# CompVis/stable-diffusion

Measured on AMD Instinct MI355X. Metric: 512x512 images/sec, SD-v1-4 50-step PLMS CFG=7.5, higher is better.
Workload: dtype f16

## Files before the change

### include/sdmi.h

```cpp
#ifndef SDMI_H_
#define SDMI_H_

#include <stdint.h>

#ifdef __cplusplus
extern "C" {
#endif

#define SDMI_ABI_VERSION 17

typedef struct sdmi_unet sdmi_unet;

typedef struct sdmi_unet_cfg {
  int32_t in_channels;
  int32_t out_channels;
  int32_t model_channels;
  int32_t num_res_blocks;
  int32_t n_levels;
  int32_t channel_mult[8];
  int32_t n_attention_resolutions;
  int32_t attention_resolutions[8];
  int32_t num_heads;
  int32_t transformer_depth;
  int32_t context_dim;
// ... 111 lines not shown
  void* pgn_out; int32_t pgn_keep_f32; int32_t* pgn_applied;
  void* out_lo;
} sdmi_igemm_desc;
int sdmi_k_igemm(const sdmi_igemm_desc* d, void* stream);
int sdmi_k_ff_tail(const sdmi_igemm_desc* proj_out, const void* ln_f16, const float* lnp, float ln_eps, const float* csd,
                   const void* wgg_f16, const void* wff2_f16, const float* bff2, const float* t, void* stream);
int sdmi_k_st_tail(const sdmi_igemm_desc* proj_out, const void* a_f16, const void* wo_f16, const float* bo, float* t, const float* ln_gamma,
                   float ln_eps, const float* csd, const void* wgg_f16, const void* wff2_f16, const float* bff2, void* stream);
int sdmi_k_gn_conv3(const sdmi_igemm_desc* conv, const float* x0, const float* x1, int c0, int c1, float* gn_ws, int64_t gn_ws_floats,
                    const float* gn_gamma, const float* gn_beta, float gn_eps, void* stream);
int sdmi_k_st_head(const float* x, float* gn_ws, int64_t gn_ws_floats, const float* gn_gamma, const float* gn_beta, float gn_eps,
                   const void* w_in3, const float* b_in, float* t, const float* ln_gamma, float ln_eps, const void* wqkv_f16,
                   const float* lnf_cs, const float* lnf_d, void* q, void* k, void* vt, int B, int ntok, int ntok_pad, int heads, int dh,
                   int C, void* stream);
int sdmi_k_st_mid(const void* a_f16, const void* wo_f16, const float* bo, float* t, const float* ln_gamma, float ln_eps, const void* wq_f16,
                  const float* lnf_cs, const float* lnf_d, void* q, int B, int ntok, int heads, int dh, int C, void* stream);
int sdmi_k_st_mid_ctx(const void* a_f16, const void* wo_f16, const float* bo, float* t, const float* ln_gamma, float ln_eps, const void* wq_f16,
                      const float* lnf_cs, const float* lnf_d, const void* ctx_k, const void* ctx_vt, int nkv, int nkv_pad, float scale, void* ao_out,
                      int B, int ntok, int heads, int dh, int C, void* stream);
int sdmi_k_ln_fold_prep(const void* w_f16, int N, int K, int ldw, const float* gamma, const float* beta, const float* bias,
                        float* cs, float* d, void* stream);
int sdmi_k_attention(const void* q, const void* k, const void* vt, void* out, int BH, int heads, int nq, int nkv,
                     int nkv_pad, int d, float scale, void* stream);
int sdmi_k_attention_ctx(const void* x, const void* wq, const void* k, const void* vt, void* out, int BH, int heads, int nq,
                         int nkv, int nkv_pad, int d, float scale, const float* lnf_part, float lnf_eps, const float* lnf_cs,
                         const float* lnf_d, void* stream);
int sdmi_k_attention_split16(const void* q, const void* q_lo, const void* k, const void* k_lo, const void* vt, const void* vt_lo, void* out,
                             void* out_lo, int BH, int heads, int nq, int nkv, int nkv_pad, int d, float scale, void* stream);
int sdmi_k_attention_causal(const void* q, const void* k, const void* vt, void* out, int BH, int heads, int n, int n_pad,
                            int d, float scale, void* stream);
int sdmi_k_groupnorm(const float* x0, const float* x1, int c0, int c1, int B, int HW, const float* gamma,
                     const float* beta, float eps, int silu, void* out_f16, float* out_f32, void* raw_f16, void* out_lo,
                     void* raw_lo, float* partial_ws, int64_t partial_floats, void* stream);
int64_t sdmi_k_groupnorm_ws_floats(int B, int HW);
int sdmi_k_conv3gn(const float* x0, const float* x1, int c0, int c1, int B, int H, int W, const float* gamma,
                   const float* beta, float eps, const void* w_packed, int N, const float* bias, const float* rowvec,
                   int ld_rowvec, const float* residual, int ldr, float* out, int ldo, int splitk, float* splitk_ws,
                   int64_t splitk_ws_floats, float* gn_ws, int64_t gn_ws_floats, int tile, void* raw_hi, void* raw_lo,
                   void* stream);
int sdmi_k_layernorm(const float* x, const float* gamma, const float* beta, void* out_f16, int M, int C, float eps,
                     void* stream);
int sdmi_k_cast_f16(const float* x, void* out_f16, void* out_lo, int64_t n, void* stream);
int sdmi_k_split_heads(const float* src, int ld, int col0, void* dst, void* dst_lo, int kind, int B, int ntok, int ntok_pad, int heads, int dh,
                       void* stream);
int sdmi_k_geglu_split(const float* src, int M, int F, void* out, void* out_lo, void* stream);
int sdmi_k_layernorm_split(const float* x, const float* gamma, const float* beta, void* out, void* out_lo, int M, int C, float eps, void* stream);
// ... 31 lines not shown
```

### stable-diffusion_amd/_lib.py

```python
import ctypes as C
import os

_HERE = os.path.dirname(os.path.abspath(__file__))
LIB_PATH = os.environ.get('SDMI_LIB_PATH') or os.path.join(_HERE, 'libsdmi.so')

c_f32p = C.c_void_p
c_ptr = C.c_void_p


class UNetCfg(C.Structure):
    _fields_ = [('in_channels', C.c_int32), ('out_channels', C.c_int32), ('model_channels', C.c_int32),
                ('num_res_blocks', C.c_int32), ('n_levels', C.c_int32), ('channel_mult', C.c_int32 * 8),
                ('n_attention_resolutions', C.c_int32), ('attention_resolutions', C.c_int32 * 8),
                ('num_heads', C.c_int32), ('transformer_depth', C.c_int32), ('context_dim', C.c_int32)]


class VaeCfg(C.Structure):
    _fields_ = [('ch', C.c_int32), ('out_ch', C.c_int32), ('n_levels', C.c_int32), ('ch_mult', C.c_int32 * 8),
                ('num_res_blocks', C.c_int32), ('in_channels', C.c_int32), ('z_channels', C.c_int32),
                ('embed_dim', C.c_int32)]


class ClipCfg(C.Structure):
    _fields_ = [('vocab_size', C.c_int32), ('hidden_size', C.c_int32), ('intermediate_size', C.c_int32),
# ... 66 lines not shown
    'sdmi_clip_set_weight': (C.c_int, [c_ptr, C.c_char_p, c_ptr, C.POINTER(C.c_int64), C.c_int, c_ptr]),
    'sdmi_clip_finalize': (C.c_int, [c_ptr]),
    'sdmi_clip_workspace_bytes': (C.c_int64, [c_ptr, C.c_int, C.c_int]),
    'sdmi_clip_forward': (C.c_int, [c_ptr, c_ptr, c_ptr, C.c_int, C.c_int, c_ptr, C.c_int64, c_ptr]),
    'sdmi_has_experiments': (C.c_int, []),
    'sdmi_k_igemm': (C.c_int, [C.POINTER(IGemmDesc), c_ptr]),
    'sdmi_k_ff_tail': (C.c_int, [C.POINTER(IGemmDesc), c_ptr, c_ptr, C.c_float, c_ptr, c_ptr, c_ptr, c_ptr, c_ptr, c_ptr]),
    'sdmi_k_gn_conv3': (C.c_int, [C.POINTER(IGemmDesc), c_ptr, c_ptr, C.c_int, C.c_int, c_ptr, C.c_int64, c_ptr, c_ptr, C.c_float, c_ptr]),
    'sdmi_k_st_mid_ctx': (C.c_int, [c_ptr, c_ptr, c_ptr, c_ptr, c_ptr, C.c_float, c_ptr, c_ptr, c_ptr, c_ptr, c_ptr, C.c_int, C.c_int, C.c_float, c_ptr,
                                    C.c_int, C.c_int, C.c_int, C.c_int, C.c_int, c_ptr]),
    'sdmi_k_st_tail': (C.c_int, [C.POINTER(IGemmDesc), c_ptr, c_ptr, c_ptr, c_ptr, c_ptr, C.c_float, c_ptr, c_ptr, c_ptr, c_ptr, c_ptr]),
    'sdmi_k_st_mid': (C.c_int, [c_ptr, c_ptr, c_ptr, c_ptr, c_ptr, C.c_float, c_ptr, c_ptr, c_ptr, c_ptr, C.c_int, C.c_int, C.c_int, C.c_int,
                                C.c_int, c_ptr]),
    'sdmi_k_st_head': (C.c_int, [c_ptr, c_ptr, C.c_int64, c_ptr, c_ptr, C.c_float, c_ptr, c_ptr, c_ptr, c_ptr, C.c_float, c_ptr, c_ptr, c_ptr,
                                 c_ptr, c_ptr, c_ptr, C.c_int, C.c_int, C.c_int, C.c_int, C.c_int, C.c_int, c_ptr]),
    'sdmi_k_attention_split16': (C.c_int, [c_ptr, c_ptr, c_ptr, c_ptr, c_ptr, c_ptr, c_ptr, c_ptr, C.c_int, C.c_int, C.c_int, C.c_int,
                                           C.c_int, C.c_int, C.c_float, c_ptr]),
    'sdmi_k_attention_causal': (C.c_int, [c_ptr, c_ptr, c_ptr, c_ptr, C.c_int, C.c_int, C.c_int, C.c_int, C.c_int, C.c_float,
                                          c_ptr]),
    'sdmi_k_pointwise_nchw': (C.c_int, [c_ptr, c_ptr, c_ptr, c_ptr, C.c_int, C.c_int, C.c_int, C.c_int, C.c_float, c_ptr]),
    'sdmi_k_softmax_rows': (C.c_int, [c_ptr, c_ptr, C.c_int, C.c_int, C.c_float, c_ptr]),
    'sdmi_k_attention': (C.c_int, [c_ptr, c_ptr, c_ptr, c_ptr, C.c_int, C.c_int, C.c_int, C.c_int, C.c_int, C.c_int,
                                   C.c_float, c_ptr]),
    'sdmi_k_groupnorm': (C.c_int, [c_ptr, c_ptr, C.c_int, C.c_int, C.c_int, C.c_int, c_ptr, c_ptr, C.c_float, C.c_int,
                                   c_ptr, c_ptr, c_ptr, c_ptr, c_ptr, c_ptr, C.c_int64, c_ptr]),
    'sdmi_k_groupnorm_ws_floats': (C.c_int64, [C.c_int, C.c_int]),
    'sdmi_k_conv3gn': (C.c_int, [c_ptr, c_ptr, C.c_int, C.c_int, C.c_int, C.c_int, C.c_int, c_ptr, c_ptr, C.c_float, c_ptr,
                                 C.c_int, c_ptr, c_ptr, C.c_int, c_ptr, C.c_int, c_ptr, C.c_int, C.c_int, c_ptr, C.c_int64,
                                 c_ptr, C.c_int64, C.c_int, c_ptr, c_ptr, c_ptr]),
    'sdmi_k_layernorm': (C.c_int, [c_ptr, c_ptr, c_ptr, c_ptr, C.c_int, C.c_int, C.c_float, c_ptr]),
    'sdmi_k_cast_f16': (C.c_int, [c_ptr, c_ptr, c_ptr, C.c_int64, c_ptr]),
    'sdmi_k_split_heads': (C.c_int, [c_ptr, C.c_int, C.c_int, c_ptr, c_ptr, C.c_int, C.c_int, C.c_int, C.c_int, C.c_int, C.c_int,
                                     c_ptr]),
    'sdmi_k_geglu_split': (C.c_int, [c_ptr, C.c_int, C.c_int, c_ptr, c_ptr, c_ptr]),
    'sdmi_k_layernorm_split': (C.c_int, [c_ptr, c_ptr, c_ptr, c_ptr, c_ptr, C.c_int, C.c_int, C.c_float, c_ptr]),
    'sdmi_k_timestep_embedding': (C.c_int, [c_ptr, c_ptr, c_ptr, C.c_int, C.c_int, c_ptr]),
    'sdmi_k_small_linear': (C.c_int, [c_ptr, C.c_int, c_ptr, c_ptr, c_ptr, C.c_int, C.c_int, C.c_int, C.c_int,
                                      C.c_int, c_ptr]),
    'sdmi_k_conv_in': (C.c_int, [c_ptr, c_ptr, c_ptr, c_ptr, C.c_int, C.c_int, C.c_int, C.c_int, C.c_int, c_ptr]),
    'sdmi_k_conv_out': (C.c_int, [c_ptr, c_ptr, c_ptr, c_ptr, C.c_int, C.c_int, C.c_int, C.c_int, C.c_int, c_ptr]),
    'sdmi_k_pack_conv_weight': (C.c_int, [c_ptr, c_ptr, C.c_int, C.c_int, C.c_int, C.c_int, c_ptr]),
    'sdmi_k_pack_conv_out': (C.c_int, [c_ptr, c_ptr, C.c_int, C.c_int, c_ptr]),
    'sdmi_k_pack_split3': (C.c_int, [c_ptr, c_ptr, C.c_int, C.c_int, c_ptr]),
    'sdmi_k_pack_geglu': (C.c_int, [c_ptr, c_ptr, c_ptr, c_ptr, C.c_int, C.c_int, c_ptr]),
    'sdmi_k_attention_ctx': (C.c_int, [c_ptr, c_ptr, c_ptr, c_ptr, c_ptr, C.c_int, C.c_int, C.c_int, C.c_int, C.c_int, C.c_int, C.c_float,
                                       c_ptr, C.c_float, c_ptr, c_ptr, c_ptr]),
# ... 55 lines not shown
```

### stable-diffusion_amd/csrc/api.cpp

```cpp
#include <string.h>

#include <new>

#include "prof.h"
#include "split16.h"
#include "unet.h"
#include "vae.h"
#include "clip.h"

namespace sdmi {
static thread_local std::string g_err;
void set_error(const std::string& msg) { g_err = msg; }
int fail(const std::string& msg) { g_err = msg; return -1; }
}

struct sdmi_unet { sdmi::UNet impl; };
struct sdmi_vae { sdmi::Vae impl; };
struct sdmi_clip { sdmi::ClipText impl; };

using namespace sdmi;

static void* g_zero_page[16] = {nullptr};
static int zero_page(const f16** out) {
  int dev = 0;
// ... 323 lines not shown
int sdmi_k_st_mid_ctx(const void* a_f16, const void* wo_f16, const float* bo, float* t, const float* ln_gamma, float ln_eps, const void* wq_f16,
                      const float* lnf_cs, const float* lnf_d, const void* ctx_k, const void* ctx_vt, int nkv, int nkv_pad, float scale, void* ao_out,
                      int B, int ntok, int heads, int dh, int C, void* stream) {
  StHeadParams p = StHeadParams();
  p.a16 = (const f16*)a_f16; p.w_in = (const f16*)wo_f16; p.b_in = bo; p.t = t; p.ln_gamma = ln_gamma; p.ln_eps = ln_eps;
  p.wqkv = (const f16*)wq_f16; p.lnf_cs = lnf_cs; p.lnf_d = lnf_d;
  p.ctx_k = (const f16*)ctx_k; p.ctx_vt = (const f16*)ctx_vt; p.ctx_nkv = nkv; p.ctx_nkv_pad = nkv_pad; p.ctx_scale = scale; p.ao_out = (f16*)ao_out;
  SDMI_CHECK(ctx_k && ctx_vt && ao_out, "st_mid_ctx: null argument");
  p.M = B * ntok; p.B = B; p.ntok = ntok; p.ntok_pad = ntok; p.heads = heads; p.dh = dh; p.C = C;
  return launch_st_mid(p, (hipStream_t)stream);
}
int sdmi_k_ln_fold_prep(const void* w_f16, int N, int K, int ldw, const float* gamma, const float* beta, const float* bias,
                        float* cs, float* d, void* stream) {
  return launch_ln_fold_prep((const f16*)w_f16, N, K, ldw, gamma, beta, bias, cs, d, (hipStream_t)stream);
}
int sdmi_k_attention(const void* q, const void* k, const void* vt, void* out, int BH, int heads, int nq, int nkv,
                     int nkv_pad, int d, float scale, void* stream) {
  AttnParams a = AttnParams();
  a.q = (const f16*)q; a.k = (const f16*)k; a.vt = (const f16*)vt; a.out = (f16*)out;
  a.BH = BH; a.heads = heads; a.nq = nq; a.nkv = nkv; a.nkv_pad = nkv_pad; a.d = d; a.scale = scale;
  if (const char* e = getenv("SDMI_ATTN_NW")) a.nw = atoi(e);
  return launch_attention(a, (hipStream_t)stream);
}
int sdmi_k_attention_split16(const void* q, const void* q_lo, const void* k, const void* k_lo, const void* vt, const void* vt_lo, void* out,
                             void* out_lo, int BH, int heads, int nq, int nkv, int nkv_pad, int d, float scale, void* stream) {
  AttnSplitParams a = AttnSplitParams();
  a.q = (const f16*)q; a.q_lo = (const f16*)q_lo; a.k = (const f16*)k; a.k_lo = (const f16*)k_lo; a.vt = (const f16*)vt;
  a.vt_lo = (const f16*)vt_lo; a.out = (f16*)out; a.out_lo = (f16*)out_lo;
  a.BH = BH; a.heads = heads; a.nq = nq; a.nkv = nkv; a.nkv_pad = nkv_pad; a.d = d; a.scale = scale;
  return launch_attention_split16(a, (hipStream_t)stream);
}
int sdmi_k_attention_ctx(const void* x, const void* wq, const void* k, const void* vt, void* out, int BH, int heads, int nq,
                         int nkv, int nkv_pad, int d, float scale, const float* lnf_part, float lnf_eps, const float* lnf_cs,
                         const float* lnf_d, void* stream) {
  AttnCtxParams a = AttnCtxParams();
  a.x = (const f16*)x; a.wq = (const f16*)wq; a.k = (const f16*)k; a.vt = (const f16*)vt; a.out = (f16*)out;
  a.BH = BH; a.heads = heads; a.nq = nq; a.nkv = nkv; a.nkv_pad = nkv_pad; a.d = d; a.C = heads * d; a.scale = scale;
  if (lnf_part) { a.lnf_part = lnf_part; a.lnf_npart = a.C / 32; a.lnf_eps = lnf_eps; a.M = (BH / heads) * nq; a.lnf_cs = lnf_cs; a.lnf_d = lnf_d; }
  return launch_attention_ctx(a, (hipStream_t)stream);
}
int64_t sdmi_k_groupnorm_ws_floats(int B, int HW) { (void)HW; return gn_acc_words(B) * 2; }
int sdmi_k_groupnorm(const float* x0, const float* x1, int c0, int c1, int B, int HW, const float* gamma,
                     const float* beta, float eps, int silu, void* out_f16, float* out_f32, void* raw_f16, void* out_lo,
                     void* raw_lo, float* partial_ws, int64_t partial_floats, void* stream) {
  SDMI_CHECK(partial_floats >= gn_acc_words(B) * 2, "groupnorm workspace too small");
  SDMI_HIP_OK(hipMemsetAsync(partial_ws, 0, gn_acc_words(B) * sizeof(long long), (hipStream_t)stream));
// ... 117 lines not shown
```

### stable-diffusion_amd/csrc/attn.hip

```cpp
#include <type_traits>

#include "common.h"
#include "prof.h"

namespace sdmi {
namespace {

constexpr int KVT = 64;
typedef float f32x2 __attribute__((ext_vector_type(2)));
typedef _Float16 f16x2 __attribute__((ext_vector_type(2)));
typedef unsigned u32x4 __attribute__((ext_vector_type(4)));

template <int N>
__device__ __forceinline__ void wait_dma() {
  static_assert(N >= 0 && N <= 44, "add the literal");
  switch (N) {
#define SDMI_VM(k) case k: asm volatile("s_waitcnt vmcnt(" #k ")" ::: "memory"); break
    SDMI_VM(0); SDMI_VM(1); SDMI_VM(2); SDMI_VM(3); SDMI_VM(4); SDMI_VM(5); SDMI_VM(6); SDMI_VM(7); SDMI_VM(8); SDMI_VM(9);
    SDMI_VM(10); SDMI_VM(11); SDMI_VM(12); SDMI_VM(13); SDMI_VM(14); SDMI_VM(15); SDMI_VM(16); SDMI_VM(17); SDMI_VM(18);
    SDMI_VM(19); SDMI_VM(20); SDMI_VM(21); SDMI_VM(22); SDMI_VM(23); SDMI_VM(24); SDMI_VM(25); SDMI_VM(26); SDMI_VM(27);
    SDMI_VM(28); SDMI_VM(29); SDMI_VM(30); SDMI_VM(31); SDMI_VM(32); SDMI_VM(33); SDMI_VM(34); SDMI_VM(35); SDMI_VM(36);
    SDMI_VM(37); SDMI_VM(38); SDMI_VM(39); SDMI_VM(40); SDMI_VM(41); SDMI_VM(42); SDMI_VM(43); SDMI_VM(44);
#undef SDMI_VM
  }
// ... 181 lines not shown
    f16* orow = p.out + ((size_t)b * p.nq + q) * ((size_t)p.heads * D) + (size_t)head * D;
#pragma unroll
    for (int dt = 0; dt < DVT; ++dt)
#pragma unroll
      for (int r4 = 0; r4 < 4; ++r4) {
        const int dd = dt * 32 + 8 * r4 + 4 * lg;
        if (dd < D) {
          f16x4 v = {(f16)(o[dt][r4 * 4 + 0] * inv), (f16)(o[dt][r4 * 4 + 1] * inv), (f16)(o[dt][r4 * 4 + 2] * inv),
                     (f16)(o[dt][r4 * 4 + 3] * inv)};
          *(f16x4*)(orow + dd) = v;
        }
      }
  }
}

__device__ __forceinline__ void head_of_block(int& bh, int& qt) {
  const unsigned nqt = gridDim.x, total = gridDim.x * gridDim.y;
  unsigned lin = blockIdx.x + nqt * blockIdx.y;
  if ((total & 7) == 0) lin = (lin & 7) * (total >> 3) + (lin >> 3);
  bh = (int)(lin / nqt);
  qt = (int)(lin - (unsigned)bh * nqt);
}

__device__ __forceinline__ void swap_halves(float& a, float& b) {
  asm volatile("s_nop 1\n\tv_permlane32_swap_b32 %0, %1\n\ts_nop 1" : "+v"(a), "+v"(b));
}
__device__ __forceinline__ float max_across_halves(float x) {
  float a = x, b = x;
  swap_halves(a, b);
  return fmaxf(a, b);
}
__device__ __forceinline__ float sum_across_halves(float x) {
  float a = x, b = x;
  swap_halves(a, b);
  return a + b;
}

template <int D, int NW, int NS, bool CAUSAL, int ABL = 0, int KVS = 1, bool ROT = false, int TPB = 1>
__global__ void __launch_bounds__(NW * 64) attn_dma_kernel(const AttnParams p) {
#if defined(__HIP_DEVICE_COMPILE__)
  constexpr int DKS = (D + 15) / 16;
  constexpr int DVT = (D + 31) / 32;
  constexpr int NCH = (D + 63) / 64;
  constexpr int KROWS = NCH * 64, VROWS = DVT * 32;
  constexpr int STAGE = (KROWS + VROWS) * 128;
  constexpr bool ONES = VROWS > D;
  constexpr int PK = NCH * 8, PV = ONES ? D / 8 : DVT * 4, PT = PK + PV;
  static_assert(D % 8 == 0, "a DMA piece is 8 rows");
  constexpr int NWQ = NW / KVS;
  static_assert(KVS == 1 || (KVS == 2 && !CAUSAL && NW % 2 == 0), "key split: two groups, no causal mask");
  static_assert(!ROT || (KVS == 2 && NS >= 4 && ABL == 0), "rotated key group: needs the key split and a ring of four stages");
  static_assert(TPB == 1 || (TPB == 2 && NS == 4 && !ROT && ABL == 0), "two tiles per barrier: a ring of exactly four stages");
  constexpr int PPW = (PT + NWQ - 1) / NWQ;
  static_assert(NS >= 2 && KVS * NS * STAGE <= 160 * 1024, "LDS budget");
  static_assert(KVS == 1 || NWQ * (DVT * 16 + 2) * 64 * 4 <= KVS * NS * STAGE, "the hand-over of the key groups lives in the (drained) rings");

  __shared__ __attribute__((aligned(16))) unsigned char smem_all[KVS * NS * STAGE];

  const int tid = threadIdx.x, lane = tid & 63;
  const int wave_all = __builtin_amdgcn_readfirstlane(tid >> 6);
  const int grp = KVS == 1 ? 0 : wave_all / NWQ;
  const int wave = KVS == 1 ? wave_all : wave_all - grp * NWQ;
  unsigned char* const smem = smem_all + grp * (NS * STAGE);
  const int l31 = lane & 31, lg = lane >> 5;
  int bh, qt;
  head_of_block(bh, qt);
  const int q0 = qt * (32 * NWQ) + wave * 32;
  const f16* Qg = p.q + (size_t)bh * p.nq * D;
  constexpr int OOB = (int)0x80000000;
  const __amdgpu_buffer_rsrc_t rsrc_k =
      __builtin_amdgcn_make_buffer_rsrc((void*)(p.k + (size_t)bh * p.nkv * D), 0, p.nkv * D * 2, 0x00020000);
  const __amdgpu_buffer_rsrc_t rsrc_v =
      __builtin_amdgcn_make_buffer_rsrc((void*)(p.vt + (size_t)bh * D * p.nkv_pad), 0, D * p.nkv_pad * 2, 0x00020000);

  f16x8 qf[DKS];
#pragma unroll
  for (int ks = 0; ks < DKS; ++ks) {
    const int dcol = ks * 16 + lg * 8;
    f16x8 v = {0, 0, 0, 0, 0, 0, 0, 0};
    if (q0 + l31 < p.nq && dcol < D) v = *(const f16x8*)(Qg + (size_t)(q0 + l31) * D + dcol);
    qf[ks] = v;
  }

  int pv_off[PPW], pv_step[PPW], pv_row[PPW];
  bool pv_isk[PPW];
#pragma unroll
  for (int j = 0; j < PPW; ++j) {
    const int q = min(wave + j * NWQ, PT - 1);
    const int r8 = lane >> 3, cp = lane & 7;
    if (q < PK) {
      const int c = q >> 3, row = (q & 7) * 8 + r8;
      const int key = (row & ~12) | ((row & 4) << 1) | ((row & 8) >> 1);
      const int gch = cp ^ ((row >> 1) & 7);
      pv_off[j] = key * (D * 2) + c * 128 + gch * 16;
// ... 15 lines not shown
    for (int j = 0; j < PPW; ++j) {
      auto dst = (__attribute__((address_space(3))) void*)(smem + stage * STAGE + pv_row[j] * 128);
      if (pv_isk[j]) __builtin_amdgcn_raw_ptr_buffer_load_lds(rsrc_k, dst, 16, pv_off[j], 0, 0, 0);
      else __builtin_amdgcn_raw_ptr_buffer_load_lds(rsrc_v, dst, 16, pv_off[j], 0, 0, 0);
      pv_off[j] += pv_step[j];
    }
  };

  f32x16 o[DVT];
#pragma unroll
  for (int dt = 0; dt < DVT; ++dt)
#pragma unroll
    for (int r = 0; r < 16; ++r) o[dt][r] = 0.f;
  float m_run = -1e30f, l_run = 0.f;
  if (ONES) {
    for (int e = tid; e < KVS * NS * (VROWS - D) * 8; e += NW * 64) {
      const int st = e / ((VROWS - D) * 8), rc = e - st * ((VROWS - D) * 8), row = D + (rc >> 3);
      const unsigned one2 = row == D ? 0x3C003C00u : 0u;
      *(u32x4*)(smem_all + st * STAGE + (KROWS + row) * 128 + (rc & 7) * 16) = u32x4{one2, one2, one2, one2};
    }
  }
  const float sc = p.scale * 1.4426950408889634f;

  const int nt_all = (p.nkv + KVT - 1) / KVT;
  const int nt = nt_all / KVS;
  const int t_first = grp * nt;
  if (KVS > 1) {
#pragma unroll
    for (int j = 0; j < PPW; ++j) pv_off[j] += t_first * pv_step[j];
  }
#pragma unroll
  for (int s2 = 0; s2 < (TPB == 2 ? 2 : NS - 1); ++s2) issue_tile(s2);
  const bool rot = ROT && grp == 1;
  if (TPB == 2) wait_dma<0>();
  else if (rot) wait_dma<PPW*(NS - 3 > 0 ? NS - 3 : 0)>(); else wait_dma<PPW*(NS - 2)>();
  asm volatile("s_waitcnt lgkmcnt(0)\n\ts_barrier" ::: "memory");
  const int ksw = (l31 >> 1) & 7;
  int cur = 0, nxt = NS - 1;
  f32x16 s[KVT / 32];
  auto qk_tile = [&](int stage) {
    const unsigned char* Kq = smem + (ABL == 6 ? 0 : stage) * STAGE;
    const f32x16 zero16 = {0.f, 0.f, 0.f, 0.f, 0.f, 0.f, 0.f, 0.f, 0.f, 0.f, 0.f, 0.f, 0.f, 0.f, 0.f, 0.f};
#pragma unroll
    for (int kvb = 0; kvb < KVT / 32; ++kvb) {
      if (ABL == 5) {
#pragma unroll
        for (int r = 0; r < 16; ++r) s[kvb][r] = 0.f;
      }
#pragma unroll
      for (int ks = 0; ks < DKS; ++ks) {
        const unsigned char* kp = Kq + ((ks >> 2) * 64 + kvb * 32 + l31) * 128 + ((((ks & 3) * 2 + lg) ^ ksw) << 4);
        const f16x8 a = *(const f16x8*)kp;
        if (ABL == 5) { s[kvb][ks] += (float)a[0]; continue; }
        s[kvb] = __builtin_amdgcn_mfma_f32_32x32x16_f16(a, qf[ks], ks == 0 ? zero16 : s[kvb], 0, 0, 0);
      }
    }
  };
  if (rot) qk_tile(0);
  if (NW == 8 && p.prio && wave >= 4) __builtin_amdgcn_s_setprio(1);
  for (int t = 0; t < nt; ++t) {
    if (TPB == 2) {
      if ((t & 1) == 0) { issue_tile((cur + 2) & 3); issue_tile((cur + 3) & 3); }
    } else if (ABL != 2) issue_tile(nxt);
    const unsigned char* Ks = smem + (ABL == 6 ? 0 : cur) * STAGE;
    const unsigned char* Vs = Ks + KROWS * 128;

    if (!rot) qk_tile(cur);
    const int kv0 = (t_first + t) * KVT;
    if (CAUSAL || kv0 + KVT > p.nkv) {
      asm volatile("; masked tile" ::: "memory");
      const int qlim = CAUSAL ? (q0 + l31) : 0x7fffffff;
#pragma unroll
      for (int kvb = 0; kvb < KVT / 32; ++kvb)
#pragma unroll
        for (int r = 0; r < 16; ++r) {
          const int kv = kv0 + kvb * 32 + (r & 3) + 4 * ((r >> 2) & 1) + 8 * lg + 16 * (r >> 3);
          if (kv >= p.nkv || kv > qlim) s[kvb][r] = -1e30f;
        }
    }
    float mx = -1e30f;
#pragma unroll
    for (int kvb = 0; kvb < KVT / 32; ++kvb)
#pragma unroll
      for (int r = 0; r < 16; ++r) mx = fmaxf(mx, s[kvb][r]);
    mx = max_across_halves(mx);
    const float m_new = fmaxf(m_run, mx * sc);
// ... 26 lines not shown
    for (int kvb = 0; kvb < KVT / 32; ++kvb) {
#pragma unroll
      for (int s2 = 0; s2 < 2; ++s2) {
        f16x8 pf;
#pragma unroll
        for (int e = 0; e < 8; ++e) pf[e] = (f16)s[kvb][8 * s2 + e];
        const int ch = 4 * kvb + 2 * s2;
#pragma unroll
        for (int dt = 0; dt < DVT; ++dt) {
          const f16x8 a = *(const f16x8*)(Vs + (dt * 32 + l31) * 128 + (((ch + lg) ^ ksw) << 4));
          if (ABL == 4) { o[dt][kvb * 2 + s2] += (float)a[0] * (float)pf[0]; continue; }
          o[dt] = __builtin_amdgcn_mfma_f32_32x32x16_f16(a, pf, o[dt], 0, 0, 0);
        }
      }
    }
    if (rot && t + 1 < nt) qk_tile((cur + 1 == NS) ? 0 : cur + 1);
    if (TPB == 2) {
      if ((t & 1) || t + 1 == nt) {
        wait_dma<0>();
        asm volatile("s_waitcnt lgkmcnt(0)\n\ts_barrier" ::: "memory");
      }
    } else if (ABL != 1) {
      if (rot) wait_dma<PPW*(NS - 3 > 0 ? NS - 3 : 0)>();
      else wait_dma<PPW*(NS - 2)>();
      asm volatile("s_waitcnt lgkmcnt(0)\n\ts_barrier" ::: "memory");
    }
    cur = (cur + 1 == NS) ? 0 : cur + 1;
    nxt = (nxt + 1 == NS) ? 0 : nxt + 1;
  }
  wait_dma<0>();

  if constexpr (KVS == 2) {
    asm volatile("s_waitcnt lgkmcnt(0)\n\ts_barrier" ::: "memory");
    float* const xch = (float*)smem_all + (size_t)wave * ((DVT * 16 + 2) * 64) + lane;
    if (grp == 1) {
#pragma unroll
      for (int dt = 0; dt < DVT; ++dt)
#pragma unroll
        for (int r = 0; r < 16; ++r) xch[(dt * 16 + r) * 64] = o[dt][r];
      xch[(DVT * 16) * 64] = m_run;
      xch[(DVT * 16 + 1) * 64] = l_run;
    }
    asm volatile("s_waitcnt lgkmcnt(0)\n\ts_barrier" ::: "memory");
    if (grp == 1) return;
    const float m1 = xch[(DVT * 16) * 64], l1 = xch[(DVT * 16 + 1) * 64];
    const float m = fmaxf(m_run, m1);
    const float a0 = __builtin_amdgcn_exp2f(m_run - m), a1 = __builtin_amdgcn_exp2f(m1 - m);
#pragma unroll
    for (int dt = 0; dt < DVT; ++dt)
#pragma unroll
      for (int r = 0; r < 16; ++r) o[dt][r] = a0 * o[dt][r] + a1 * xch[(dt * 16 + r) * 64];
    l_run = a0 * l_run + a1 * l1;
  }

  float l_tot;
  if (ONES) {
    constexpr int rl = D % 32, r_l = (rl & 3) + 4 * (rl >> 3), lg_l = (rl >> 2) & 1;
    float a = o[D / 32][r_l], b = a;
    swap_halves(a, b);
    l_tot = lg_l == 0 ? a : b;
  } else {
    l_tot = sum_across_halves(l_run);
  }
  const float inv = 1.0f / l_tot;
  const int q = q0 + l31;
  if (q < p.nq) {
    const int b = bh / p.heads, head = bh - b * p.heads;
    f16* orow = p.out + ((size_t)b * p.nq + q) * ((size_t)p.heads * D) + (size_t)head * D;
#pragma unroll
    for (int dt = 0; dt < DVT; ++dt)
#pragma unroll
      for (int r4 = 0; r4 < 4; ++r4) {
        const int dd = dt * 32 + 8 * r4 + 4 * lg;
        if (dd < D) {
          f16x4 v = {(f16)(o[dt][r4 * 4 + 0] * inv), (f16)(o[dt][r4 * 4 + 1] * inv), (f16)(o[dt][r4 * 4 + 2] * inv),
                     (f16)(o[dt][r4 * 4 + 3] * inv)};
          SDMI_ST(f16x4, orow + dd, v);
        }
      }
  }
#endif
}

#ifdef SDMI_EXPERIMENTS
template <int D, int NS>
__global__ void __launch_bounds__(512) attn_pp_kernel(const AttnParams p) {
#if defined(__HIP_DEVICE_COMPILE__)
  constexpr int NW = 8;
  constexpr int DKS = (D + 15) / 16;
  constexpr int DVT = (D + 31) / 32;
  constexpr int NCH = (D + 63) / 64;
  constexpr int KROWS = NCH * 64, VROWS = DVT * 32;
  constexpr int STAGE = (KROWS + VROWS) * 128;
  constexpr bool ONES = VROWS > D;
  constexpr int PK = NCH * 8, PV = ONES ? D / 8 : DVT * 4, PT = PK + PV;
  static_assert(D % 8 == 0, "a DMA piece is 8 rows");
  constexpr int PPW = (PT + NW - 1) / NW;
  static_assert(NS >= 4 && NS * STAGE <= 160 * 1024, "LDS budget (the ring runs NS - 2 tiles ahead)");

  __shared__ __attribute__((aligned(16))) unsigned char smem[NS * STAGE];

  const int tid = threadIdx.x, lane = tid & 63;
  const int wave = __builtin_amdgcn_readfirstlane(tid >> 6);
  const int grp = wave >> 2;
// ... 204 lines not shown
          SDMI_ST(f16x4, orow + dd, v);
        }
      }
  }
#endif
}
#endif

#ifdef SDMI_EXPERIMENTS
#define SDMI_EXP_ENV(name, def) (getenv(name) ? atoi(getenv(name)) : (def))
#else
#define SDMI_EXP_ENV(name, def) (def)
#endif

#ifndef SDMI_ATTN_TPB_DEFAULT
#define SDMI_ATTN_TPB_DEFAULT 1
#endif
#ifndef SDMI_ATTN_ROT_DEFAULT
#define SDMI_ATTN_ROT_DEFAULT 0
#endif
#ifndef SDMI_ATTN_KVS_DEFAULT
#define SDMI_ATTN_KVS_DEFAULT 1
#endif
template <int D>
int launch_d(const AttnParams& p, hipStream_t stream) {
  int nw = p.nw;
  if (nw <= 0) {
    const int slices = cdiv(p.nq, 32);
    nw = (slices >= 8 && p.nq > 1024) ? 8 : (slices >= 4 ? 4 : 2);
    static const int env_small = SDMI_EXP_ENV("SDMI_ATTN_NW_LE1K", 0);
    static const int env_big = SDMI_EXP_ENV("SDMI_ATTN_NW_GT1K", 0);
    if (env_small > 0 && p.nq <= 1024) nw = env_small;
    if (env_big > 0 && p.nq > 1024) nw = env_big;
  }
  dim3 grid(cdiv(p.nq, 32 * nw), p.BH);
  static const std::string pname_long = std::string("attn_d") + std::to_string(D) + "_self";
  static const std::string pname_short = std::string("attn_d") + std::to_string(D) + "_ctx";
  ProfScope ps((p.nkv >= 256 ? pname_long : pname_short).c_str(), 4.0 * p.BH * (double)p.nq * p.nkv * D, 2.0 * p.BH * D * (2.0 * p.nq + 2.0 * p.nkv), stream);
  static const int use_v1 = SDMI_EXP_ENV("SDMI_ATTN_V1", 0);
  constexpr int DNS = (D > 128) ? 3 : 4;
  const int kvs_env = getenv("SDMI_ATTN_KVS") ? atoi(getenv("SDMI_ATTN_KVS")) : SDMI_ATTN_KVS_DEFAULT;
  const bool tpb2 = SDMI_EXP_ENV("SDMI_ATTN_TPB", SDMI_ATTN_TPB_DEFAULT) == 2;
  const bool kvs_rot = SDMI_EXP_ENV("SDMI_ATTN_ROT", SDMI_ATTN_ROT_DEFAULT) != 0;
  (void)tpb2; (void)kvs_rot;
  const bool kvs2 = D == 40 && nw == 8 && !p.causal && !p.pingpong && p.nkv % (2 * KVT) == 0 && p.nkv >= 32 * KVT && kvs_env != 0 && (p.nkv <= 64 * KVT || kvs_env == 2);
  if (!use_v1 && !p.causal && (p.nkv * D) % 8 == 0) {
#ifdef SDMI_ABLATE
    static const int abl = getenv("SDMI_ATTN_ABL") ? atoi(getenv("SDMI_ATTN_ABL")) : 0;
// ... 75 lines not shown
```

### stable-diffusion_amd/csrc/common.h

```cpp
#pragma once
#include <hip/hip_runtime.h>
#include <stdint.h>
#include <algorithm>
#include <string>

#include "tape.h"

typedef _Float16 f16;
typedef _Float16 f16x2 __attribute__((ext_vector_type(2)));
typedef _Float16 f16x4 __attribute__((ext_vector_type(4)));
typedef _Float16 f16x8 __attribute__((ext_vector_type(8)));
typedef float f32x4 __attribute__((ext_vector_type(4)));
typedef float f32x16 __attribute__((ext_vector_type(16)));

#ifdef __HIPCC__
__device__ __forceinline__ float gn_apply_elem(float v, float mean, float rstd, float gamma, float beta, int silu) {
  float t = __builtin_fmaf((v - mean) * rstd, gamma, beta);
  if (silu) t = t * __builtin_amdgcn_rcpf(1.0f + __expf(-t));
  return t;
}
__device__ __forceinline__ void gn_acc_add(unsigned long long* dst, float v) {
  const double d = (double)v;
  const double hi = rint(d);
  atomicAdd(dst, (unsigned long long)(long long)hi);
// ... 216 lines not shown
  const float* x0 = nullptr; const float* x1 = nullptr; int c0 = 0, c1 = 0;
  const long long* gn_acc = nullptr;
  const float* gn_gamma = nullptr; const float* gn_beta = nullptr; float gn_eps = 1e-5f;
  const f16* w = nullptr;
#ifdef SDMI_RC_TIMING
  long long* dbg = nullptr;
#endif
  IGemmParams epi;
};
bool gn_conv3_supported(int B, int H, int W, int c0, int c1, int Cout);
int launch_gn_conv3(const GnConvParams& p, hipStream_t stream);

struct AttnParams {
  const f16* q = nullptr;
  const f16* k = nullptr;
  const f16* vt = nullptr;
  f16* out = nullptr;
  int BH = 0, heads = 0, nq = 0, nkv = 0, nkv_pad = 0, d = 0;
  float scale = 1.f;
  int nw = 0;
  int causal = 0;
  int prio = 0;
  int pingpong = 0;
};
int launch_attention(const AttnParams& p, hipStream_t stream);

struct AttnCtxParams {
  const f16* x = nullptr;
  const f16* wq = nullptr;
  const f16* k = nullptr;
  const f16* vt = nullptr;
  f16* out = nullptr;
  int BH = 0, heads = 0, nq = 0, nkv = 0, nkv_pad = 0, d = 0, C = 0;
  float scale = 1.f;
  const float* lnf_part = nullptr; int lnf_npart = 0; float lnf_eps = 1e-5f; int M = 0;
  const float* lnf_cs = nullptr; const float* lnf_d = nullptr;
};
bool attention_ctx_supported(int d, int C, int nkv);
int launch_attention_ctx(const AttnCtxParams& p, hipStream_t stream);

struct GroupNormParams {
  const float* x0 = nullptr; const float* x1 = nullptr; int c0 = 0, c1 = 0;
  int B = 0, HW = 0;
  const float* gamma = nullptr; const float* beta = nullptr; float eps = 1e-5f;
  int silu = 0;
  int stats_only = 0;
// ... 78 lines not shown
```

### stable-diffusion_amd/csrc/unet.cpp

```cpp
#include "unet.h"

extern "C" char** environ;
#include "prof.h"
#include "split16.h"

#include <math.h>
#include <stdio.h>
#include <string.h>

#include <algorithm>

namespace sdmi {

static bool in_list(const int* v, int n, int x) {
  for (int i = 0; i < n; ++i)
    if (v[i] == x) return true;
  return false;
}

void UNet::expect(const std::string& key, std::vector<int64_t> shape, WKind kind, void** dst, int row0, int ld,
                  void** dst2) {
  WeightSlot s;
  s.key = key; s.shape = std::move(shape); s.kind = kind; s.dst = dst; s.row0 = row0; s.ld = ld; s.dst2 = dst2;
  slot_index_[key] = (int)slots_.size();
// ... 828 lines not shown
      p.Hout = H * W;
      p.bias = L.f32[3]; p.residual = x.p; p.ldr = C; p.out_f32 = out.p; p.ldo = C;
      attach_gn_targets(p, out);
      attach_f16_copy(p, out);
      if (chain_ff) {
        TBlock& T = L.tb[0];
        FfTailParams q = FfTailParams();
        q.ln = ln; q.lnp = lnp; q.ln_eps = 1e-5f; q.csd = T.lnf_csd; q.wgg = T.wgg; q.wff2 = T.wff2; q.bff2 = T.bff2; q.t = t; q.wpo = L.w16[1];
        if (chain_tail) { q.a16 = ao; q.wo = T.wo2; q.bo = T.bo2; q.ln_gamma = T.ln[4]; }
        q.epi = p;
        if (!dry && !rc) ok(launch_ff_tail(q, s));
      } else {
        gemm(p);
      }
    }
    scratch.off = mark;
    return out;
  }

  void attention(const f16* q, const f16* k, const f16* vt, f16* out, Layer& L, int nq, int nkv, int nkv_pad, float scale) {
    AttnParams a = AttnParams();
    a.q = q; a.k = k; a.vt = vt; a.out = out; a.BH = B * L.heads; a.heads = L.heads; a.nq = nq; a.nkv = nkv;
    a.nkv_pad = nkv_pad; a.d = L.dh; a.scale = scale;
    if (!dry && !rc) ok(launch_attention(a, s));
  }

  Act resample(Layer& L, const Act& x, bool up) {
    const int Hin = x.H, Win = x.W, C = x.C;
    const int Hout = up ? 2 * Hin : (Hin - 1) / 2 + 1, Wout = up ? 2 * Win : (Win - 1) / 2 + 1;
    const size_t mark = scratch.off;
    if (u->full()) {
      const int64_t n = (int64_t)B * Hin * Win * C;
      f16* hi = S<f16>((size_t)n); f16* lo = S<f16>((size_t)n);
      if (!dry && !rc) ok(launch_cast_f16(x.p, hi, lo, n, s));
      Act out = make_act(P<float>((size_t)B * Hout * Wout * C), L.cout, Hout, Wout, true);
      IGemmParams p = conv3(hi, C, Hin, Win, Hout, Wout, up ? 1 : 2, up ? 1 : 0, L.w16[0], L.cout);
      p.a1 = lo; p.c1 = C; p.lda1 = C; p.a2 = hi; p.c2 = C; p.lda2 = C; p.K = 27 * C; p.k_alg = 9 * C;
      p.bias = L.f32[0]; p.out_f32 = out.p; p.ldo = L.cout;
      attach_gn_targets(p, out);
      gemm(p);
      scratch.off = mark;
      return out;
    }
    const f16* x16 = nullptr;
    if (dry) { if (!want_f16_copy(x)) (void)S<f16>((size_t)B * Hin * Win * C); }
    else {
// ... 349 lines not shown
```

Before: 3.807.

## Add split-KV attention path with combine kernel and default key split

Adds a split-KV variant of the DMA attention kernel. Key tiles are divided into chunks spread over a third grid dimension, and each chunk writes unnormalised partial outputs plus its running max and sum to a workspace. A separate combine kernel then merges them with log-sum-exp weighting. For non-causal attention with at most 1024 queries, the default plan now picks the in-workgroup two-group key split when the tile count is even and at least eight, and otherwise the single-chunk SKV kernel. The aim is more parallelism for the small low-resolution attention calls. The cost is extra workspace traffic and an extra launch when chunking is enabled, plus different wave counts from the previous heuristic.

```diff
diff --git a/include/sdmi.h b/include/sdmi.h
--- a/include/sdmi.h
+++ b/include/sdmi.h
@@ -157,6 +157,8 @@
                         float* cs, float* d, void* stream);
 int sdmi_k_attention(const void* q, const void* k, const void* vt, void* out, int BH, int heads, int nq, int nkv,
                      int nkv_pad, int d, float scale, void* stream);
+int sdmi_k_attention_ws(const void* q, const void* k, const void* vt, void* out, int BH, int heads, int nq, int nkv,
+                        int nkv_pad, int d, float scale, float* ws, int64_t ws_floats, void* stream);
 int sdmi_k_attention_ctx(const void* x, const void* wq, const void* k, const void* vt, void* out, int BH, int heads, int nq,
                          int nkv, int nkv_pad, int d, float scale, const float* lnf_part, float lnf_eps, const float* lnf_cs,
                          const float* lnf_d, void* stream);
diff --git a/stable-diffusion_amd/_lib.py b/stable-diffusion_amd/_lib.py
--- a/stable-diffusion_amd/_lib.py
+++ b/stable-diffusion_amd/_lib.py
@@ -112,6 +112,8 @@
     'sdmi_k_softmax_rows': (C.c_int, [c_ptr, c_ptr, C.c_int, C.c_int, C.c_float, c_ptr]),
     'sdmi_k_attention': (C.c_int, [c_ptr, c_ptr, c_ptr, c_ptr, C.c_int, C.c_int, C.c_int, C.c_int, C.c_int, C.c_int,
                                    C.c_float, c_ptr]),
+    'sdmi_k_attention_ws': (C.c_int, [c_ptr, c_ptr, c_ptr, c_ptr, C.c_int, C.c_int, C.c_int, C.c_int, C.c_int, C.c_int,
+                                      C.c_float, c_ptr, C.c_int64, c_ptr]),
     'sdmi_k_groupnorm': (C.c_int, [c_ptr, c_ptr, C.c_int, C.c_int, C.c_int, C.c_int, c_ptr, c_ptr, C.c_float, C.c_int,
                                    c_ptr, c_ptr, c_ptr, c_ptr, c_ptr, c_ptr, C.c_int64, c_ptr]),
     'sdmi_k_groupnorm_ws_floats': (C.c_int64, [C.c_int, C.c_int]),
diff --git a/stable-diffusion_amd/csrc/api.cpp b/stable-diffusion_amd/csrc/api.cpp
--- a/stable-diffusion_amd/csrc/api.cpp
+++ b/stable-diffusion_amd/csrc/api.cpp
@@ -369,6 +369,14 @@
   if (const char* e = getenv("SDMI_ATTN_NW")) a.nw = atoi(e);
   return launch_attention(a, (hipStream_t)stream);
 }
+int sdmi_k_attention_ws(const void* q, const void* k, const void* vt, void* out, int BH, int heads, int nq, int nkv,
+                        int nkv_pad, int d, float scale, float* ws, int64_t ws_floats, void* stream) {
+  AttnParams a = AttnParams();
+  a.q = (const f16*)q; a.k = (const f16*)k; a.vt = (const f16*)vt; a.out = (f16*)out;
+  a.BH = BH; a.heads = heads; a.nq = nq; a.nkv = nkv; a.nkv_pad = nkv_pad; a.d = d; a.scale = scale;
+  a.ws = ws; a.ws_floats = ws_floats;
+  return launch_attention(a, (hipStream_t)stream);
+}
 int sdmi_k_attention_split16(const void* q, const void* q_lo, const void* k, const void* k_lo, const void* vt, const void* vt_lo, void* out,
                              void* out_lo, int BH, int heads, int nq, int nkv, int nkv_pad, int d, float scale, void* stream) {
   AttnSplitParams a = AttnSplitParams();
diff --git a/stable-diffusion_amd/csrc/attn.hip b/stable-diffusion_amd/csrc/attn.hip
--- a/stable-diffusion_amd/csrc/attn.hip
+++ b/stable-diffusion_amd/csrc/attn.hip
@@ -1,3 +1,5 @@
+#include <stdio.h>
+
 #include <type_traits>
 
 #include "common.h"
@@ -227,6 +229,16 @@
   qt = (int)(lin - (unsigned)bh * nqt);
 }
 
+__device__ __forceinline__ void skv_block(int& bh, int& qt, int& chunk) {
+  const unsigned nqt = gridDim.x, ns = gridDim.z, total = gridDim.x * gridDim.y * gridDim.z;
+  unsigned lin = blockIdx.x + nqt * (blockIdx.y + gridDim.y * blockIdx.z);
+  if ((total & 7) == 0) lin = (lin & 7) * (total >> 3) + (lin >> 3);
+  qt = (int)(lin % nqt);
+  const unsigned r = lin / nqt;
+  chunk = (int)(r % ns);
+  bh = (int)(r / ns);
+}
+
 __device__ __forceinline__ void swap_halves(float& a, float& b) {
   asm volatile("s_nop 1\n\tv_permlane32_swap_b32 %0, %1\n\ts_nop 1" : "+v"(a), "+v"(b));
 }
@@ -241,7 +253,7 @@
   return a + b;
 }
 
-template <int D, int NW, int NS, bool CAUSAL, int ABL = 0, int KVS = 1, bool ROT = false, int TPB = 1>
+template <int D, int NW, int NS, bool CAUSAL, int ABL = 0, int KVS = 1, bool ROT = false, int TPB = 1, bool SKV = false>
 __global__ void __launch_bounds__(NW * 64) attn_dma_kernel(const AttnParams p) {
 #if defined(__HIP_DEVICE_COMPILE__)
   constexpr int DKS = (D + 15) / 16;
@@ -257,7 +269,9 @@
   static_assert(!ROT || (KVS == 2 && NS >= 4 && ABL == 0), "rotated key group: needs the key split and a ring of four stages");
   static_assert(TPB == 1 || (TPB == 2 && NS == 4 && !ROT && ABL == 0), "two tiles per barrier: a ring of exactly four stages");
   constexpr int PPW = (PT + NWQ - 1) / NWQ;
-  static_assert(NS >= 2 && KVS * NS * STAGE <= 160 * 1024, "LDS budget");
+  static_assert((NS >= 2 || (SKV && KVS == 1 && TPB == 1 && ABL == 0)) && KVS * NS * STAGE <= 160 * 1024, "LDS budget");
+  static_assert(!SKV || (KVS == 1 && !CAUSAL && ABL == 0 && TPB == 1), "split-KV: one key group per workgroup, no causal mask");
+  constexpr int WAIT_NEXT = NS >= 2 ? PPW * (NS - 2) : 0;
   static_assert(KVS == 1 || NWQ * (DVT * 16 + 2) * 64 * 4 <= KVS * NS * STAGE, "the hand-over of the key groups lives in the (drained) rings");
 
   __shared__ __attribute__((aligned(16))) unsigned char smem_all[KVS * NS * STAGE];
@@ -268,13 +282,18 @@
   const int wave = KVS == 1 ? wave_all : wave_all - grp * NWQ;
   unsigned char* const smem = smem_all + grp * (NS * STAGE);
   const int l31 = lane & 31, lg = lane >> 5;
-  int bh, qt;
-  head_of_block(bh, qt);
+  int bh, qt, chunk = 0;
+  if constexpr (SKV) skv_block(bh, qt, chunk);
+  else head_of_block(bh, qt);
   const int q0 = qt * (32 * NWQ) + wave * 32;
   const f16* Qg = p.q + (size_t)bh * p.nq * D;
   constexpr int OOB = (int)0x80000000;
+  const int nt_all = (p.nkv + KVT - 1) / KVT;
+  const int nt = SKV ? min(p.skv_tpc, nt_all - chunk * p.skv_tpc) : nt_all / KVS;
+  const int t_first = SKV ? chunk * p.skv_tpc : grp * nt;
+  const int k_end = SKV ? min(p.nkv, (t_first + nt) * KVT) : p.nkv;
   const __amdgpu_buffer_rsrc_t rsrc_k =
-      __builtin_amdgcn_make_buffer_rsrc((void*)(p.k + (size_t)bh * p.nkv * D), 0, p.nkv * D * 2, 0x00020000);
+      __builtin_amdgcn_make_buffer_rsrc((void*)(p.k + (size_t)bh * p.nkv * D), 0, k_end * D * 2, 0x00020000);
   const __amdgpu_buffer_rsrc_t rsrc_v =
       __builtin_amdgcn_make_buffer_rsrc((void*)(p.vt + (size_t)bh * D * p.nkv_pad), 0, D * p.nkv_pad * 2, 0x00020000);
 
@@ -336,18 +355,15 @@
   }
   const float sc = p.scale * 1.4426950408889634f;
 
-  const int nt_all = (p.nkv + KVT - 1) / KVT;
-  const int nt = nt_all / KVS;
-  const int t_first = grp * nt;
-  if (KVS > 1) {
+  if (KVS > 1 || SKV) {
 #pragma unroll
     for (int j = 0; j < PPW; ++j) pv_off[j] += t_first * pv_step[j];
   }
 #pragma unroll
-  for (int s2 = 0; s2 < (TPB == 2 ? 2 : NS - 1); ++s2) issue_tile(s2);
+  for (int s2 = 0; s2 < (TPB == 2 ? 2 : NS > 1 ? NS - 1 : 1); ++s2) issue_tile(s2);
   const bool rot = ROT && grp == 1;
   if (TPB == 2) wait_dma<0>();
-  else if (rot) wait_dma<PPW*(NS - 3 > 0 ? NS - 3 : 0)>(); else wait_dma<PPW*(NS - 2)>();
+  else if (rot) wait_dma<PPW*(NS - 3 > 0 ? NS - 3 : 0)>(); else wait_dma<WAIT_NEXT>();
   asm volatile("s_waitcnt lgkmcnt(0)\n\ts_barrier" ::: "memory");
   const int ksw = (l31 >> 1) & 7;
   int cur = 0, nxt = NS - 1;
@@ -375,7 +391,7 @@
   for (int t = 0; t < nt; ++t) {
     if (TPB == 2) {
       if ((t & 1) == 0) { issue_tile((cur + 2) & 3); issue_tile((cur + 3) & 3); }
-    } else if (ABL != 2) issue_tile(nxt);
+    } else if (ABL != 2 && NS > 1) issue_tile(nxt);
     const unsigned char* Ks = smem + (ABL == 6 ? 0 : cur) * STAGE;
     const unsigned char* Vs = Ks + KROWS * 128;
 
@@ -448,7 +464,7 @@
       }
     } else if (ABL != 1) {
       if (rot) wait_dma<PPW*(NS - 3 > 0 ? NS - 3 : 0)>();
-      else wait_dma<PPW*(NS - 2)>();
+      else wait_dma<WAIT_NEXT>();
       asm volatile("s_waitcnt lgkmcnt(0)\n\ts_barrier" ::: "memory");
     }
     cur = (cur + 1 == NS) ? 0 : cur + 1;
@@ -488,6 +504,22 @@
   } else {
     l_tot = sum_across_halves(l_run);
   }
+  if (SKV && p.skv_s > 1) {
+    const int q = q0 + l31;
+    if (q < p.nq) {
+      const size_t row = ((size_t)chunk * p.BH + bh) * p.nq + q;
+      float* orow = p.ws + row * D;
+#pragma unroll
+      for (int dt = 0; dt < DVT; ++dt)
+#pragma unroll
+        for (int r4 = 0; r4 < 4; ++r4) {
+          const int dd = dt * 32 + 8 * r4 + 4 * lg;
+          if (dd < D) *(f32x4*)(orow + dd) = f32x4{o[dt][r4 * 4 + 0], o[dt][r4 * 4 + 1], o[dt][r4 * 4 + 2], o[dt][r4 * 4 + 3]};
+        }
+      if (lg == 0) *(f32x2*)(p.ws + (size_t)p.skv_s * p.BH * p.nq * D + 2 * row) = f32x2{m_run, l_tot};
+    }
+    return;
+  }
   const float inv = 1.0f / l_tot;
   const int q = q0 + l31;
   if (q < p.nq) {
@@ -506,6 +538,35 @@
       }
   }
 #endif
+}
+
+template <int D>
+__global__ void __launch_bounds__(256) attn_skv_combine(const AttnParams p) {
+  constexpr int DG = D / 4;
+  const int64_t rows = (int64_t)p.BH * p.nq;
+  const int64_t i = (int64_t)blockIdx.x * 256 + threadIdx.x;
+  if (i >= rows * DG) return;
+  const int64_t row = i / DG;
+  const int g = (int)(i - row * DG);
+  const int S = p.skv_s;
+  const f32x2* ml = (const f32x2*)(p.ws + (size_t)S * rows * D);
+  float m = -1e30f;
+  for (int s = 0; s < S; ++s) m = fmaxf(m, ml[s * rows + row][0]);
+  f32x4 acc = {0.f, 0.f, 0.f, 0.f};
+  float l = 0.f;
+  for (int s = 0; s < S; ++s) {
+    const f32x2 e = ml[s * rows + row];
+    const float w = __builtin_amdgcn_exp2f(e[0] - m);
+    l = fmaf(w, e[1], l);
+    const f32x4 o = *(const f32x4*)(p.ws + ((size_t)s * rows + row) * D + 4 * g);
+#pragma unroll
+    for (int j = 0; j < 4; ++j) acc[j] = fmaf(w, o[j], acc[j]);
+  }
+  const float inv = 1.0f / l;
+  const int bh = (int)(row / p.nq), q = (int)(row - (int64_t)bh * p.nq);
+  const int b = bh / p.heads, head = bh - b * p.heads;
+  f16* orow = p.out + ((size_t)b * p.nq + q) * ((size_t)p.heads * D) + (size_t)head * D + 4 * g;
+  SDMI_ST(f16x4, orow, (f16x4{(f16)(acc[0] * inv), (f16)(acc[1] * inv), (f16)(acc[2] * inv), (f16)(acc[3] * inv)}));
 }
 
 #ifdef SDMI_EXPERIMENTS
@@ -756,8 +817,82 @@
 #ifndef SDMI_ATTN_KVS_DEFAULT
 #define SDMI_ATTN_KVS_DEFAULT 1
 #endif
+struct SkvPlan { int s = 1, nw = 2, ns = 1, tpc = 1, kvs = 1; };
+static int64_t skv_ws_need(const AttnParams& p, int s) { return s > 1 ? (int64_t)s * p.BH * p.nq * (p.d + 2) : 0; }
+static int attn_stage_bytes(int D) { return ((D + 63) / 64 * 64 + (D + 31) / 32 * 32) * 128; }
+static SkvPlan skv_plan(const AttnParams& p, const char* cfg) {
+  SkvPlan k;
+  const int nt = cdiv(p.nkv, KVT);
+  int s_req = 1, ns_req = 0, nw = 0, kvs = 1;
+  if (cfg && *cfg) {
+    if (sscanf(cfg, "%d,%d,%d,%d", &s_req, &nw, &ns_req, &kvs) >= 2 && (nw == 2 || nw == 4 || (kvs == 2 && nw == 8))) k.nw = nw;
+    if (kvs == 2 && nt % 2 == 0 && 2 * 2 * attn_stage_bytes(p.d) <= 160 * 1024) {
+      k.kvs = 2; k.ns = 2; k.nw = std::max(k.nw, 4);
+      return k;
+    }
+  } else if (nt % 2 == 0 && nt >= 8 && 2 * 2 * attn_stage_bytes(p.d) <= 160 * 1024) {
+    k.kvs = 2; k.nw = 4; k.ns = 2;
+    return k;
+  }
+  s_req = std::max(1, std::min(s_req, nt));
+  while (s_req > 1 && (p.ws == nullptr || skv_ws_need(p, s_req) > p.ws_floats)) --s_req;
+  k.tpc = cdiv(nt, s_req);
+  k.s = cdiv(nt, k.tpc);
+  k.ns = (ns_req >= 1 && ns_req <= 3) ? std::min(ns_req, std::max(k.tpc, 2)) : std::min(k.tpc, 3);
+  if (k.tpc > 1 && k.ns < 2) k.ns = 2;
+  return k;
+}
+template <int D, int NW>
+void skv_launch_nw(const AttnParams& p, int ns, dim3 grid, hipStream_t stream) {
+  if (ns == 1) SDMI_LAUNCH((attn_dma_kernel<D, NW, 1, false, 0, 1, false, 1, true>), grid, dim3(NW * 64), 0, stream, p);
+  else if (ns == 2) SDMI_LAUNCH((attn_dma_kernel<D, NW, 2, false, 0, 1, false, 1, true>), grid, dim3(NW * 64), 0, stream, p);
+  else SDMI_LAUNCH((attn_dma_kernel<D, NW, 3, false, 0, 1, false, 1, true>), grid, dim3(NW * 64), 0, stream, p);
+}
+template <int D>
+int launch_skv(const AttnParams& p_in, const SkvPlan& k, hipStream_t stream) {
+  AttnParams p = p_in;
+  p.skv_s = k.s; p.skv_tpc = k.tpc;
+  if (k.kvs == 2) {
+    if constexpr (2 * 2 * (((D + 63) / 64 * 64 + (D + 31) / 32 * 32) * 128) <= 160 * 1024) {
+      static const std::string pname_long = std::string("attn_d") + std::to_string(D) + "_self";
+      static const std::string pname_short = std::string("attn_d") + std::to_string(D) + "_ctx";
+      ProfScope ps((p.nkv >= 256 ? pname_long : pname_short).c_str(), 4.0 * p.BH * (double)p.nq * p.nkv * D,
+                   2.0 * p.BH * D * (2.0 * p.nq + 2.0 * p.nkv), stream);
+      const dim3 grid(cdiv(p.nq, 32 * (k.nw / 2)), p.BH);
+      if (k.nw == 8) SDMI_LAUNCH((attn_dma_kernel<D, 8, 2, false, 0, 2>), grid, dim3(512), 0, stream, p);
+      else SDMI_LAUNCH((attn_dma_kernel<D, 4, 2, false, 0, 2>), grid, dim3(256), 0, stream, p);
+      SDMI_HIP_OK(hipGetLastError());
+      return 0;
+    }
+    return fail("attention: no in-workgroup key split at this head dim");
+  }
+  SDMI_CHECK(k.s == 1 || (p.ws && ((uintptr_t)p.ws & 15) == 0 && skv_ws_need(p, k.s) <= p.ws_floats), "split-KV attention: bad workspace");
+  const dim3 grid(cdiv(p.nq, 32 * k.nw), p.BH, k.s);
+  {
+    static const std::string pname_long = std::string("attn_d") + std::to_string(D) + "_self";
+    static const std::string pname_short = std::string("attn_d") + std::to_string(D) + "_ctx";
+    const double bytes = 2.0 * p.BH * D * (2.0 * p.nq + 2.0 * p.nkv) + (k.s > 1 ? 4.0 * skv_ws_need(p, k.s) - 2.0 * p.BH * p.nq * D : 0.0);
+    ProfScope ps((p.nkv >= 256 ? pname_long : pname_short).c_str(), 4.0 * p.BH * (double)p.nq * p.nkv * D, bytes, stream);
+    if (k.nw == 2) skv_launch_nw<D, 2>(p, k.ns, grid, stream);
+    else skv_launch_nw<D, 4>(p, k.ns, grid, stream);
+    SDMI_HIP_OK(hipGetLastError());
+  }
+  if (k.s > 1) {
+    static const std::string pname_comb = std::string("attn_d") + std::to_string(D) + "_combine";
+    const int64_t threads = (int64_t)p.BH * p.nq * (D / 4);
+    ProfScope ps(pname_comb.c_str(), 0.0, 4.0 * skv_ws_need(p, k.s) + 2.0 * p.BH * p.nq * D, stream);
+    SDMI_LAUNCH((attn_skv_combine<D>), dim3((unsigned)((threads + 255) / 256)), dim3(256), 0, stream, p);
+    SDMI_HIP_OK(hipGetLastError());
+  }
+  return 0;
+}
+
 template <int D>
 int launch_d(const AttnParams& p, hipStream_t stream) {
+  if (!p.causal && p.nw <= 0 && p.nq <= 1024 && (p.nkv * D) % 8 == 0) {
+    const char* e = getenv("SDMI_ATTN_SPLITKV");
+    if (!(e && atoi(e) == 0)) return launch_skv<D>(p, skv_plan(p, getenv("SDMI_ATTN_SKV_CFG")), stream);
+  }
   int nw = p.nw;
   if (nw <= 0) {
     const int slices = cdiv(p.nq, 32);
diff --git a/stable-diffusion_amd/csrc/common.h b/stable-diffusion_amd/csrc/common.h
--- a/stable-diffusion_amd/csrc/common.h
+++ b/stable-diffusion_amd/csrc/common.h
@@ -262,6 +262,8 @@
   int causal = 0;
   int prio = 0;
   int pingpong = 0;
+  int skv_s = 1, skv_tpc = 0;
+  float* ws = nullptr; int64_t ws_floats = 0;
 };
 int launch_attention(const AttnParams& p, hipStream_t stream);
 
diff --git a/stable-diffusion_amd/csrc/unet.cpp b/stable-diffusion_amd/csrc/unet.cpp
--- a/stable-diffusion_amd/csrc/unet.cpp
+++ b/stable-diffusion_amd/csrc/unet.cpp
@@ -874,6 +874,7 @@
     AttnParams a = AttnParams();
     a.q = q; a.k = k; a.vt = vt; a.out = out; a.BH = B * L.heads; a.heads = L.heads; a.nq = nq; a.nkv = nkv;
     a.nkv_pad = nkv_pad; a.d = L.dh; a.scale = scale;
+    a.ws = splitk_ws; a.ws_floats = splitk_ws_floats;
     if (!dry && !rc) ok(launch_attention(a, s));
   }
 
```

After: 3.824, median of 6. About the same (+0.4%).
